# adityamwagh/SuperSLAM

Measured on AMD Instinct MI355X. Metric: stereo pairs/sec (SPx2+LG) at 1376x376, higher is better.
Workload: dtype f16; 1 GPU; configs[1]: SuperPoint x2 + select + gather + 1x LightGlue on 1376x376 stereo pairs; a step = 8 x 64 = 512 pairs per GPU resident in HBM (8 library calls of 64 pairs, different images per call), max_keypoints 600, seeded synthetic weights; pairs_per_call=64, max_keypoints=600, matches_last_call=1412, parallelism=replicated weights, pairs sharded over 1 rank(s), no data-path collective

## Files before the change

superslam_amd/csrc/api.hip:

```cpp
#include <algorithm>
#include <atomic>
#include <cmath>
#include <cstdarg>
#include <cstdlib>
#include <cstring>
#include <fstream>
#include <map>
#include <memory>
#include <mutex>
#include <string>
#include <vector>

#include "../../include/sship.h"
#include "../../include/superslam_hip/place_recognizer.hpp"
#include "kernels.h"

namespace sship {

static thread_local std::string g_err;
static void (*g_log_cb)(int, const char*) = nullptr;
static int g_profiling = 0;

void set_error(const std::string& msg) {
  g_err = msg;
// ... 508 lines not shown
  float* b1a = nullptr;
  _Float16* w1a_frag = nullptr;
  _Float16* w1a_fragb = nullptr;
  ConvW c1b, c2a, c2b, c3a, c3b, c4a, c4b, cPa, cPb, cDa, cDb;
  ConvW cDb32;
  sship_pool* pool = nullptr;
  int wsB = 0, wsH = 0, wsW = 0;
  DevBuf img, a1a, a1b, a2a, a2b, a3a, a3b, a4a, a4b, aPa, aDa, draw, logits, cand, cand_count;
  const void* cand_zero_ptr = nullptr; int cand_zero_n = 0;
  hipStream_t cand_zero_stream = nullptr;
  DevBuf kp, cell_h, cell_w, n_dev, desc_stage, gray_in;
  PinBuf h_kp, h_n, h_img;
  int cap = 0;
  float thr_f = 0.f;
  bool img_valid = false;
  struct Ring {
    int depth = 0, h = 0, w = 0, ch = 0;
    size_t img_bytes = 0;
    std::vector<void*> host, dev;
    std::vector<hipEvent_t> uploaded;
    hipStream_t copy_stream = nullptr;
    struct Pending { bool active = false; int slots[2] = {-1, -1}; int rc_pool = 0; hipEvent_t done = nullptr; void* h_kp = nullptr; void* h_n = nullptr; };
    std::vector<Pending> pending;
  } ring;
};

static void ring_free(sship_sp* sp);
static void sp_shapes(int H, int W, int& H2, int& W2, int& H4, int& W4, int& Hc, int& Wc) {
  H2 = H / 2; W2 = W / 2; H4 = H2 / 2; W4 = W2 / 2; Hc = H4 / 2; Wc = W4 / 2;
}

static int sp_ensure(sship_sp* sp, int B, int H, int W) {
  if (B <= sp->wsB && H == sp->wsH && W == sp->wsW) return SSHIP_OK;
  int H2, W2, H4, W4, Hc, Wc;
  sp_shapes(H, W, H2, W2, H4, W4, Hc, Wc);
  if (Hc < 1 || Wc < 1) return fail(SSHIP_ERR_INVALID, "image too small for SuperPoint (needs >= 8x8)");
  const size_t px1 = (size_t)B * H * W, px2 = (size_t)B * H2 * W2, px4 = (size_t)B * H4 * W4, pxc = (size_t)B * Hc * Wc;
  const int mk = sp->cfg.max_keypoints;
  SSHIP_HIP_CHECK(sp->img.ensure(px1));
  SSHIP_HIP_CHECK(sp->gray_in.ensure(px1 * 3));
  SSHIP_HIP_CHECK(sp->a1a.ensure(px1 * 64 * 2));
  SSHIP_HIP_CHECK(sp->a1b.ensure(px2 * 64 * 2));
  SSHIP_HIP_CHECK(sp->a2a.ensure(px2 * 64 * 2));
  SSHIP_HIP_CHECK(sp->a2b.ensure(px4 * 64 * 2));
  SSHIP_HIP_CHECK(sp->a3a.ensure(px4 * 128 * 2));
  SSHIP_HIP_CHECK(sp->a3b.ensure(pxc * 128 * 2));
  SSHIP_HIP_CHECK(sp->a4a.ensure(pxc * 128 * 2));
  SSHIP_HIP_CHECK(sp->a4b.ensure(pxc * 128 * 2));
  SSHIP_HIP_CHECK(sp->aPa.ensure(pxc * 256 * 2));
  SSHIP_HIP_CHECK(sp->aDa.ensure(pxc * 256 * 2));
  SSHIP_HIP_CHECK(sp->draw.ensure(pxc * 256 * 2));
  SSHIP_HIP_CHECK(sp->logits.ensure(pxc * kLogitStride * 4));
  sp->cap = Hc * 8 * Wc * 8;
  SSHIP_HIP_CHECK(sp->cand.ensure((size_t)B * sp->cap * 8));
  SSHIP_HIP_CHECK(sp->cand_count.ensure((size_t)B * 4));
  SSHIP_HIP_CHECK(sp->kp.ensure((size_t)B * mk * 3 * 4));
  SSHIP_HIP_CHECK(sp->cell_h.ensure((size_t)B * mk * 4));
  SSHIP_HIP_CHECK(sp->cell_w.ensure((size_t)B * mk * 4));
  SSHIP_HIP_CHECK(sp->n_dev.ensure((size_t)B * 4));
  SSHIP_HIP_CHECK(sp->h_kp.ensure((size_t)B * mk * 3 * 4));
  SSHIP_HIP_CHECK(sp->h_n.ensure((size_t)B * 4));
  SSHIP_HIP_CHECK(sp->h_img.ensure(px1 * 3));
  sp->wsB = B; sp->wsH = H; sp->wsW = W;
  return SSHIP_OK;
// ... 3 lines not shown
  static const int v = [] {
    const char* e = dev_env("SUPERSLAM_HIP_CONV");
    return (SSHIP_DEV_SWITCHES && e && std::string(e) == "strip") ? 2 : 1;
  }();
  return v;
}
static hipError_t conv3(const ConvW& w, const _Float16* in, _Float16* out, int B, int H, int W, bool pool, hipStream_t s) {
#if SSHIP_DEV_SWITCHES
  static const bool wino = [] { const char* e = dev_env("SUPERSLAM_HIP_CONV64"); return e && std::string(e) == "wino"; }();
  if (wino && w.w_wino && sp_conv3x3_wino_fits(H, W, w.cin, w.cout)) return sp_conv3x3_wino(w.w_wino, w.bias, in, out, B, H, W, pool, s);
  return conv_mode() == 1 ? sp_conv3x3_pp(w, in, out, B, H, W, pool, s) : sp_conv3x3_strip(w, in, out, B, H, W, pool, s);
#else
  return sp_conv3x3_pp(w, in, out, B, H, W, pool, s);
#endif
}
static bool conv2_fused(int B, int H2, int W2) {
#if SSHIP_DEV_SWITCHES
  static const std::string mode = [] { const char* e = dev_env("SUPERSLAM_HIP_CONV2"); return std::string(e ? e : ""); }();
  static const bool other = [] { const char* e = dev_env("SUPERSLAM_HIP_CONV64"); return e != nullptr; }();
  if (mode == "split" || other || conv_mode() != 1) return false;
#endif
  return sp_conv2ab_fused_fits(B, H2, W2, true);
}
static hipError_t conv3a_layer(const ConvW& w, const _Float16* in, _Float16* out, int B, int H, int W, hipStream_t s) {
#if SSHIP_DEV_SWITCHES
  static const bool roll = [] { const char* e = dev_env("SUPERSLAM_HIP_CONV3A"); return e && std::string(e) == "roll"; }();
  if (roll && conv_mode() == 1 && w.cin == 64 && w.cout == 128 && w.ct == 64 && sp_conv3a_roll_fits(B, H, W)) return sp_conv3a_roll(w, in, out, B, H, W, s);
#endif
  return conv3(w, in, out, B, H, W, false, s);
}
// ... 24 lines not shown
    g_timer.mark_fine("sp_gpu_infer:encoder/conv2a+conv2b+pool", s);
  } else {
    SSHIP_HIP_CHECK(conv3(sp->c2a, sp->a1b.as<_Float16>(), sp->a2a.as<_Float16>(), B, H2, W2, false, s));
    g_timer.mark_fine("sp_gpu_infer:encoder/conv2a", s);
    SSHIP_HIP_CHECK(conv3(sp->c2b, sp->a2a.as<_Float16>(), sp->a2b.as<_Float16>(), B, H2, W2, true, s));
    g_timer.mark_fine("sp_gpu_infer:encoder/conv2b+pool", s);
  }
  SSHIP_HIP_CHECK(conv3a_layer(sp->c3a, sp->a2b.as<_Float16>(), sp->a3a.as<_Float16>(), B, H4, W4, s));
  g_timer.mark_fine("sp_gpu_infer:encoder/conv3a", s);
  SSHIP_HIP_CHECK(conv3(sp->c3b, sp->a3a.as<_Float16>(), sp->a3b.as<_Float16>(), B, H4, W4, true, s));
  g_timer.mark_fine("sp_gpu_infer:encoder/conv3b+pool", s);
  SSHIP_HIP_CHECK(conv3(sp->c4a, sp->a3b.as<_Float16>(), sp->a4a.as<_Float16>(), B, Hc, Wc, false, s));
  g_timer.mark_fine("sp_gpu_infer:encoder/conv4a", s);
  SSHIP_HIP_CHECK(conv3(sp->c4b, sp->a4a.as<_Float16>(), sp->a4b.as<_Float16>(), B, Hc, Wc, false, s));
  g_timer.mark(g_profiling >= 2 ? "sp_gpu_infer:encoder/conv4b" : "sp_gpu_infer:encoder", s);
  SSHIP_HIP_CHECK(conv3(sp->cPa, sp->a4b.as<_Float16>(), sp->aPa.as<_Float16>(), B, Hc, Wc, false, s));
  g_timer.mark_fine("sp_gpu_infer:heads/convPa", s);
  SSHIP_HIP_CHECK(sp_conv1x1_f32(sp->cPb, sp->aPa.as<_Float16>(), sp->logits.as<float>(), kLogitStride, B, Hc, Wc, s));
  if (dense_desc || desc_dense_mode()) SSHIP_HIP_CHECK(conv3(sp->cDa, sp->a4b.as<_Float16>(), sp->aDa.as<_Float16>(), B, Hc, Wc, false, s));
  if (dense_desc) SSHIP_HIP_CHECK(sp_conv1x1_f16(sp->cDb, sp->aDa.as<_Float16>(), sp->draw.as<_Float16>(), B, Hc, Wc, s));
  g_timer.mark(g_profiling >= 2 ? "sp_gpu_infer:heads/convPb" : "sp_gpu_infer:heads", s);
  return SSHIP_OK;
}

static int sp_select(sship_sp* sp, int B, int H, int W, float* scores_out, float* kp_out, int* n_out, hipStream_t s) {
  int H2, W2, H4, W4, Hc, Wc;
  sp_shapes(H, W, H2, W2, H4, W4, Hc, Wc);
  if (sp->cand_zero_ptr != sp->cand_count.p || sp->cand_zero_n < B || sp->cand_zero_stream != s)
    SSHIP_HIP_CHECK(hipMemsetAsync(sp->cand_count.p, 0, (size_t)B * 4, s));
  sp->cand_zero_ptr = sp->cand_count.p; sp->cand_zero_n = 0; sp->cand_zero_stream = s;
  NmsArgs a{};
  a.logits = sp->logits.as<float>(); a.ls = kLogitStride; a.B = B; a.H = Hc * 8; a.W = Wc * 8;
  a.radius = sp->cfg.nms_radius; a.thr_f = sp->thr_f; a.border = sp->cfg.remove_borders;
  a.cand = sp->cand.as<unsigned long long>(); a.cand_count = sp->cand_count.as<int>(); a.cap = sp->cap;
  a.scores_out = scores_out;
  launch_nms_tile(0, a, s);
// ... 178 lines not shown
  SSHIP_HIP_CHECK(mfma_probe(random_operands != 0, tflops));
  return SSHIP_OK;
}

extern "C" int sship_sp_bench_layer(sship_sp* sp, int layer, int batch, int h, int w, int iters, float* avg_ms,
                                    double* macs) {
  bind_thread();
  if (!sp || !avg_ms || iters <= 0 || layer < 0 || layer > 15) return fail(SSHIP_ERR_INVALID, "sp_bench_layer: bad arguments");
  if (batch > sp->wsB || h != sp->wsH || w != sp->wsW) return fail(SSHIP_ERR_INVALID, "sp_bench_layer: run the network at this shape first");
  if (layer <= 1 && !sp->img_valid)
    return fail(SSHIP_ERR_INVALID, "sp_bench_layer: the handle holds no copy of the last input - make one call with sship_set_profiling(1) first "
                                   "(a launch on stale / zero pixels runs at a higher clock than the real one)");
  int H2, W2, H4, W4, Hc, Wc;
  sp_shapes(h, w, H2, W2, H4, W4, Hc, Wc);
  hipStream_t s = sp->stream;
  _Float16 *a1a = sp->a1a.as<_Float16>(), *a1b = sp->a1b.as<_Float16>(), *a2a = sp->a2a.as<_Float16>(),
           *a2b = sp->a2b.as<_Float16>(), *a3a = sp->a3a.as<_Float16>(), *a3b = sp->a3b.as<_Float16>(),
           *a4a = sp->a4a.as<_Float16>(), *a4b = sp->a4b.as<_Float16>(), *aPa = sp->aPa.as<_Float16>(),
           *aDa = sp->aDa.as<_Float16>();
  auto run = [&]() -> hipError_t {
    switch (layer) {
      case 0: launch_conv1a(sp->img.as<uint8_t>(), sp->w1a, sp->b1a, a1a, batch, h, w, s); return hipGetLastError();
      case 1: return conv1ab(sp, sp->img.as<uint8_t>(), a1b, batch, h, w, s);
      case 15:
        if (!sp_conv2ab_fused_fits(batch, H2, W2, true)) return hipErrorInvalidValue;
        return sp_conv2ab_fused(sp->c2a, sp->c2b, a1b, a2b, batch, H2, W2, s);
      case 2: return conv3(sp->c2a, a1b, a2a, batch, H2, W2, false, s);
      case 3: return conv3(sp->c2b, a2a, a2b, batch, H2, W2, true, s);
      case 4: return conv3a_layer(sp->c3a, a2b, a3a, batch, H4, W4, s);
      case 5: return conv3(sp->c3b, a3a, a3b, batch, H4, W4, true, s);
      case 6: return conv3(sp->c4a, a3b, a4a, batch, Hc, Wc, false, s);
      case 7: return conv3(sp->c4b, a4a, a4b, batch, Hc, Wc, false, s);
      case 8: return conv3(sp->cPa, a4b, aPa, batch, Hc, Wc, false, s);
      case 9: return sp_conv1x1_f32(sp->cPb, aPa, sp->logits.as<float>(), kLogitStride, batch, Hc, Wc, s);
      case 10: return conv3(sp->cDa, a4b, aDa, batch, Hc, Wc, false, s);
      case 11: return sp_conv1x1_f16(sp->cDb, aDa, sp->draw.as<_Float16>(), batch, Hc, Wc, s);
      case 12: {
        if (hipError_t e = hipMemsetAsync(sp->cand_count.p, 0, (size_t)batch * 4, s)) return e;
        sp->cand_zero_n = 0;
        NmsArgs a{};
        a.logits = sp->logits.as<float>(); a.ls = kLogitStride; a.B = batch; a.H = Hc * 8; a.W = Wc * 8;
        a.radius = sp->cfg.nms_radius; a.thr_f = sp->thr_f; a.border = sp->cfg.remove_borders;
        a.cand = sp->cand.as<unsigned long long>(); a.cand_count = sp->cand_count.as<int>(); a.cap = sp->cap;
        launch_nms_tile(0, a, s);
        return hipGetLastError();
      }
      case 13: {
        TopkArgs t{};
// ... 1010 lines not shown
```

superslam_amd/csrc/conv_pp128.hip:

```cpp
#include "igemm.h"
#include "kernels.h"

#include <cstdio>
#include <cstdlib>
#include <string>
#include <type_traits>
#include <vector>

#ifndef SSHIP_PP_PRIO
#define SSHIP_PP_PRIO 2
#endif
#ifndef SSHIP_PP_TRACE_BUILD
#define SSHIP_PP_TRACE_BUILD 0
#endif

#ifndef SSHIP_PP128_ABL
#define SSHIP_PP128_ABL 0
#endif
#ifndef SSHIP_PP128_COLMAJOR
#define SSHIP_PP128_COLMAJOR 0
#endif

namespace sship {

struct Pp128Args {
  const _Float16* in;
  const _Float16* wpack;
  const float* bias;
  _Float16* out;
  int B, H, W, cout;
  unsigned long long* trace;
  int pairs_on;
};

constexpr int Q_TH = 8, Q_TW = 32, Q_THH = 10, Q_TWH = 34;
constexpr int Q_IN_HALFS = Q_THH * Q_TWH * 32;
constexpr int Q_W_SLOT = 9 * 2 * 2 * 512;
constexpr int Q_ROW_UNITS = Q_TWH * 4;
constexpr int Q_NCHUNK = 4;
constexpr unsigned Q_OOB = 0xfffffff0u;

__device__ __forceinline__ int pp128_lds(int row, int col, int unit) {
  return (row * Q_TWH + col) * 32 + ((unit ^ ((col >> 2) & 3)) << 3);
}

struct TileWalk { int tx, ty, b; };

// ... 292 lines not shown
    std::vector<unsigned long long> h(4096 * 2 * 6);
    (void)hipStreamSynchronize(s);
    (void)hipMemcpy(h.data(), tbuf, h.size() * 8, hipMemcpyDeviceToHost);
    double sum[6] = {0}; long cnt = 0;
    for (int i = 0; i < gx * ncb * 2; ++i) {
      if (!h[i * 6 + 3]) continue;
      for (int k = 0; k < 6; ++k) sum[k] += (double)h[i * 6 + k];
      ++cnt;
    }
    if (cnt) fprintf(stderr, "[pp128 trace cout=%d pool=%d] weight dma issue=%.0f stage+dma wait=%.0f prefetch issue=%.0f | mfma=%.0f | barrier wait after data=%.0f after mfma=%.0f (clk, %ld groups)\n",
                     a.cout, (int)POOL, sum[0] / cnt, sum[1] / cnt, sum[2] / cnt, sum[3] / cnt, sum[4] / cnt, sum[5] / cnt, cnt);
  }
  return hipGetLastError();
}

constexpr int R_TH = 16, R_THH = 18;
constexpr int R_IN_UNITS = R_THH * Q_TWH * 4;
constexpr int R_IN_DMA = (R_IN_UNITS + 63) / 64;
constexpr int R_IN_HALFS = R_IN_DMA * 64 * 8;
constexpr int R_DMA_PER_WAVE = 10;
constexpr unsigned R_OOB = 0x80000000u;

typedef int rsrc4_t __attribute__((ext_vector_type(4)));

__host__ __device__ inline bool pp128w_pairs_shape(bool pool, int B, int W) {
  const int we = W - ((W + Q_TW - 1) / Q_TW - 1) * Q_TW;
  return !pool && (B & 1) == 0 && W > Q_TW && we >= 1 && we <= 15;
}
#define pp128w_pairs(pool, B, W) (p.pairs_on && pp128w_pairs_shape(pool, B, W))
template <bool POOL, int NCH>
__global__ __launch_bounds__(512, 2) void conv3x3_pp128w(Pp128Args p) {
  constexpr int MT = 2, NT = 4;
  constexpr int PB = NCH * 64;
  extern __shared__ __attribute__((aligned(16))) char smem128w[];
  _Float16* s_w = reinterpret_cast<_Float16*>(smem128w);
  const int tid = threadIdx.x, wave = tid >> 6, lane = tid & 63, j = lane & 31, hh = lane >> 5;
  const int grp = __builtin_amdgcn_readfirstlane(wave >> 2);
  const int gw = wave & 3;
  const int gw_u = __builtin_amdgcn_readfirstlane(gw);
  _Float16* my_in = s_w + 2 * Q_W_SLOT + grp * R_IN_HALFS;
  float* s_bias = reinterpret_cast<float*>(s_w + 2 * Q_W_SLOT + 2 * R_IN_HALFS);

  const int tiles_x = (p.W + Q_TW - 1) / Q_TW, tiles_y = (p.H + R_TH - 1) / R_TH;
  const bool pairs = pp128w_pairs(POOL, p.B, p.W);
  const int txn = tiles_x - 1, we = p.W - txn * Q_TW;
  const int tiles_xv = pairs ? 2 * txn + 1 : tiles_x, nb_walk = pairs ? p.B / 2 : p.B;
  const int ntiles = nb_walk * tiles_xv * tiles_y;
  const int cb = blockIdx.y;
  const int t_begin = (int)((long long)blockIdx.x * ntiles / gridDim.x);
  const int t_end = (int)((long long)(blockIdx.x + 1) * ntiles / gridDim.x);
  const int n_wg = t_end - t_begin;
  if (n_wg <= 0) return;
  const _Float16* wsrc = p.wpack + (size_t)cb * (NCH * Q_W_SLOT);

  for (int u = tid; u < (NCH == 2 ? 2 : 1) * Q_W_SLOT / 8; u += 512) *reinterpret_cast<uint4*>(s_w + u * 8) = *reinterpret_cast<const uint4*>(wsrc + u * 8);
  if (tid < 256) s_bias[tid] = p.bias[cb * 64 + (tid & 63)];
  const unsigned lane16 = lane * 16;
  const int dma_f0 = gw_u < 2 ? gw_u * 5 : 10 + (gw_u - 2) * 4;
  auto fill_weights = [&](int cn, int half) __attribute__((always_inline)) {
    const unsigned long long ga = (unsigned long long)(uintptr_t)(wsrc + (size_t)cn * Q_W_SLOT + (half * 18 + dma_f0) * 512);
    const unsigned long long g = (unsigned long long)(unsigned)__builtin_amdgcn_readfirstlane((unsigned)ga) |
                                 ((unsigned long long)(unsigned)__builtin_amdgcn_readfirstlane((unsigned)(ga >> 32)) << 32);
    const unsigned dst = __builtin_amdgcn_readfirstlane((unsigned)(uintptr_t)(s_w + (cn & 1) * Q_W_SLOT + (half * 18 + dma_f0) * 512));
    unsigned keep;
    asm volatile("s_mov_b32 %0, m0\n\ts_mov_b32 m0, %2\n\ts_nop 0\n\t"
                 "global_load_lds_dwordx4 %1, %3\n\t"
                 "global_load_lds_dwordx4 %1, %3 offset:1024\n\t"
                 "global_load_lds_dwordx4 %1, %3 offset:2048\n\t"
                 "global_load_lds_dwordx4 %1, %3 offset:3072\n\t"
                 "s_mov_b32 m0, %0"
                 : "=&s"(keep) : "v"(lane16), "s"(dst), "s"(g) : "memory");
// ... 75 lines not shown
    rs[3] = 0x00020000;
  }
  const unsigned lds_in0 = __builtin_amdgcn_readfirstlane((unsigned)(uintptr_t)(my_in + (gw_u * R_DMA_PER_WAVE) * 512));
  auto dma_tile = [&](const TileWalk& w, int chunk, unsigned m0a, unsigned m0b, unsigned m0c) __attribute__((always_inline)) {
    int img, txr;
    bool shared;
    decode(w, img, txr, shared);
    const int y0 = w.ty * R_TH, x0 = txr * Q_TW;
    const unsigned soff = __builtin_amdgcn_readfirstlane((unsigned)((img * p.H + y0) * p.W + x0) * (unsigned)PB + (unsigned)chunk * 64u);
    const bool interior = !shared && y0 >= 1 && y0 + R_TH + 1 <= p.H && x0 >= 1 && x0 + Q_TW + 1 <= p.W;
    unsigned v[R_DMA_PER_WAVE];
    if (interior) {
#pragma unroll
      for (int i = 0; i < R_DMA_PER_WAVE; ++i) v[i] = voff[i];
    } else if (shared) {
      unsigned ok = 0x3ffu & ~m_dead;
      if (w.ty == 0) ok &= m_top;
      if (w.ty == tiles_y - 1) ok &= m_bot;
      const unsigned delta = (unsigned)(p.H * p.W - (we + 2)) * (unsigned)PB;
#pragma unroll
      for (int i = 0; i < R_DMA_PER_WAVE; ++i) v[i] = (ok >> i) & 1u ? voff[i] + ((m_second >> i) & 1u ? delta : 0u) : R_OOB;
    } else {
      unsigned ok = 0x3ffu;
      if (w.ty == 0) ok &= m_top;
      if (w.ty == tiles_y - 1) ok &= m_bot;
      if (txr == 0) ok &= m_left;
      if (txr == tiles_x - 1) ok &= m_right;
#pragma unroll
      for (int i = 0; i < R_DMA_PER_WAVE; ++i) v[i] = (ok >> i) & 1u ? voff[i] : R_OOB;
    }
    unsigned keep;
    asm volatile("s_mov_b32 %0, m0\n\ts_mov_b32 m0, %5\n\ts_nop 0\n\t"
                 "buffer_load_dwordx4 %1, %6, %7 offen lds\n\t"
                 "buffer_load_dwordx4 %2, %6, %7 offen offset:1024 lds\n\t"
                 "buffer_load_dwordx4 %3, %6, %7 offen offset:2048 lds\n\t"
                 "buffer_load_dwordx4 %4, %6, %7 offen offset:3072 lds\n\t"
                 "s_mov_b32 m0, %0"
                 : "=&s"(keep) : "v"(v[0]), "v"(v[1]), "v"(v[2]), "v"(v[3]), "s"(m0a), "s"(rs), "s"(soff) : "memory");
    asm volatile("s_mov_b32 %0, m0\n\ts_mov_b32 m0, %5\n\ts_nop 0\n\t"
                 "buffer_load_dwordx4 %1, %6, %7 offen lds\n\t"
                 "buffer_load_dwordx4 %2, %6, %7 offen offset:1024 lds\n\t"
                 "buffer_load_dwordx4 %3, %6, %7 offen offset:2048 lds\n\t"
                 "buffer_load_dwordx4 %4, %6, %7 offen offset:3072 lds\n\t"
                 "s_mov_b32 m0, %0"
                 : "=&s"(keep) : "v"(v[4]), "v"(v[5]), "v"(v[6]), "v"(v[7]), "s"(m0b), "s"(rs), "s"(soff) : "memory");
    if (gw_u < 3)
      asm volatile("s_mov_b32 %0, m0\n\ts_mov_b32 m0, %3\n\ts_nop 0\n\t"
                   "buffer_load_dwordx4 %1, %4, %5 offen lds\n\t"
                   "buffer_load_dwordx4 %2, %4, %5 offen offset:1024 lds\n\t"
                   "s_mov_b32 m0, %0"
                   : "=&s"(keep) : "v"(v[8]), "v"(v[9]), "s"(m0c), "s"(rs), "s"(soff) : "memory");
    else
      asm volatile("s_mov_b32 %0, m0\n\ts_mov_b32 m0, %2\n\ts_nop 0\n\t"
                   "buffer_load_dwordx4 %1, %3, %4 offen lds\n\t"
                   "s_mov_b32 m0, %0"
                   : "=&s"(keep) : "v"(v[8]), "s"(m0c), "s"(rs), "s"(soff) : "memory");
  };
  auto dma_in = [&](int chunk) __attribute__((always_inline)) {
    dma_tile(pw, chunk, lds_in0, lds_in0 + 4096u, lds_in0 + 8192u);
    if (chunk == NCH - 1) walk_next(pw);
  };

  f16x_t acc[MT][NT];
  auto mfma_item = [&](auto chunk_c) __attribute__((always_inline)) {
    constexpr int chunk = decltype(chunk_c)::value;
    const _Float16* wc = s_w + (chunk & 1) * Q_W_SLOT + lane * 8;
    const _Float16* ib = my_in + (gw * 4) * Q_TWH * 32;
    h8_t af[3][MT], rows[8];
    auto load_a = [&](int s_, int buf) __attribute__((always_inline)) {
      const int t = s_ / 3, ky = s_ - 3 * t, kx = t >> 1, ksl = t & 1, idx = (ky * 3 + kx) * 2 + ksl;
#pragma unroll
      for (int m = 0; m < MT; ++m) af[buf][m] = *reinterpret_cast<const h8_t*>(wc + (idx * MT + m) * 512);
    };
    auto load_row = [&](int t, int row) __attribute__((always_inline)) {
      rows[(6 * t + row) & 7] = *reinterpret_cast<const h8_t*>(ib + row * Q_TWH * 32 + boff[t >> 1][t & 1]);
    };
#pragma unroll
    for (int row = 0; row < 4; ++row) load_row(0, row);
    load_a(0, 0);
    load_a(1, 1);
    if constexpr (chunk == 0) {
#pragma unroll
      for (int m = 0; m < MT; ++m)
#pragma unroll
        for (int n = 0; n < NT; ++n)
#pragma unroll
          for (int g = 0; g < 4; ++g) {
            const float4 b4 = *reinterpret_cast<const float4*>(s_bias + n * 64 + m * 32 + hh * 4 + g * 8);
            acc[m][n][4 * g + 0] = b4.x; acc[m][n][4 * g + 1] = b4.y; acc[m][n][4 * g + 2] = b4.z; acc[m][n][4 * g + 3] = b4.w;
          }
    }
    if constexpr ((SSHIP_PP128_ABL & 8) != 0) {
      load_a(2, 2);
#pragma unroll
      for (int row = 4; row < 8; ++row) rows[row] = rows[row - 4];
    }
#pragma unroll
    for (int s_ = 0; s_ < 18; ++s_) {
      const int t = s_ / 3, ky = s_ - 3 * t;
      if constexpr ((SSHIP_PP128_ABL & 8) == 0) {
      if (s_ + 2 < 18) load_a(s_ + 2, (s_ + 2) % 3);
      if (ky == 0) {
        load_row(t, 4); load_row(t, 5);
        if (t + 1 < 6) { load_row(t + 1, 0); load_row(t + 1, 1); }
      } else if (t + 1 < 6) load_row(t + 1, ky + 1);
      }
      __builtin_amdgcn_sched_barrier(0);
#pragma unroll
      for (int n = 0; n < NT; ++n)
#pragma unroll
        for (int m = 0; m < MT; ++m) {
          if constexpr ((SSHIP_PP128_ABL & 1) != 0) asm volatile("" :: "v"(af[s_ % 3][m]), "v"(rows[(6 * t + n + ky) & 7]));
          else acc[m][n] = mfma32(af[s_ % 3][m], rows[(6 * t + n + ky) & 7], acc[m][n]);
        }
      __builtin_amdgcn_sched_barrier(0);
    }
  };
  auto epilogue = [&]() __attribute__((always_inline)) {
    int b, txr;
    bool shared;
    decode(ew, b, txr, shared);
    const int y0 = ew.ty * R_TH, x0 = txr * Q_TW;
    walk_next(ew);
    const int yb = y0 + gw * 4;
    int x = x0 + j;
    if (shared) {
      const bool second = j >= we + 2;
      b += second;
// ... 41 lines not shown
        auto pool1 = [&](int m, int r) __attribute__((always_inline)) -> float {
          const float tt = fmaxf(fmaxf(acc[m][2 * q][r], acc[m][2 * q + 1][r]), 0.f);
          const float nb = __int_as_float(__builtin_amdgcn_update_dpp(0, __float_as_int(tt), 0xB1, 0xF, 0xF, false));
          return fmaxf(tt, nb);
        };
#pragma unroll
        for (int m = 0; m < MT; ++m)
#pragma unroll
          for (int g = 0; g < 4; g += 2)
            store_pair(pix, m, g, pack2(pool1(m, 4 * g + 0), pool1(m, 4 * g + 1)), pack2(pool1(m, 4 * g + 2), pool1(m, 4 * g + 3)),
                       pack2(pool1(m, 4 * g + 4), pool1(m, 4 * g + 5)), pack2(pool1(m, 4 * g + 6), pool1(m, 4 * g + 7)), ok);
      }
    }
  };

  const int T0 = (n_wg + 1) >> 1, T1 = n_wg >> 1;
  unsigned long long* trow = p.trace + ((size_t)(blockIdx.y * gridDim.x + blockIdx.x) * 2 + grp) * 6;
  const bool tr_lane = SSHIP_PP_TRACE_BUILD && p.trace && gw == 0 && lane == 0;
  unsigned long long t0 = 0, t1 = 0;
  auto data_role = [&](int dma_chunk, int dma_half, int in_chunk, bool tr) __attribute__((always_inline)) {
    if (SSHIP_PP_PRIO) __builtin_amdgcn_s_setprio(SSHIP_PP_PRIO);
    if (tr) t0 = __builtin_readcyclecounter();
    if constexpr ((SSHIP_PP128_ABL & 2) != 0) {
      if (in_chunk >= 0 && in_chunk == NCH - 1) walk_next(pw);
    } else {
    if (in_chunk >= 0) dma_in(in_chunk);
    if (NCH == 4 && dma_chunk >= 0) fill_weights(dma_chunk, dma_half);
    }
    if (SSHIP_PP_PRIO) __builtin_amdgcn_s_setprio(0);
    if (tr) { t1 = __builtin_readcyclecounter(); trow[0] = t1 - t0; t0 = t1; }
    asm volatile("s_waitcnt vmcnt(0)" ::: "memory");
    if (tr) { t1 = __builtin_readcyclecounter(); trow[1] = t1 - t0; trow[2] = 0; t0 = t1; }
    __syncthreads();
    if (tr) trow[4] = __builtin_readcyclecounter() - t0;
  };
  auto mfma_role = [&](auto chunk_c, bool tr) __attribute__((always_inline)) {
    constexpr int chunk = decltype(chunk_c)::value;
    if (tr) t0 = __builtin_readcyclecounter();
    mfma_item(chunk_c);
    if constexpr (chunk == NCH - 1) {
      if constexpr ((SSHIP_PP128_ABL & 4) != 0) {
        walk_next(ew);
#pragma unroll
        for (int m = 0; m < MT; ++m)
#pragma unroll
          for (int n = 0; n < NT; ++n) asm volatile("" :: "v"(acc[m][n]));
      } else epilogue();
    }
    if (tr) { t1 = __builtin_readcyclecounter(); trow[3] = t1 - t0; t0 = t1; }
    __syncthreads();
    if (tr) trow[5] = __builtin_readcyclecounter() - t0;
  };
  const std::integral_constant<int, 0> c0{};
  const std::integral_constant<int, 1> c1{};
  const std::integral_constant<int, 2> c2{};
  const std::integral_constant<int, 3> c3{};
  __syncthreads();
  if constexpr (NCH == 4) {
    if (grp == 0) {
      data_role(-1, 0, T0 > 0 ? 0 : -1, false);
#pragma unroll 1
      for (int it = 0; it < T0; ++it) {
        const bool more = it + 1 < T0, tr = tr_lane && it == 1;
        mfma_role(c0, tr);
        data_role(1, 1, 1, tr);
        mfma_role(c1, false);
        data_role(2, 1, 2, false);
        mfma_role(c2, false);
        data_role(3, 1, 3, false);
        mfma_role(c3, false);
        data_role(0, 1, more ? 0 : -1, false);
      }
    } else {
// ... 76 lines not shown
    std::vector<unsigned long long> h(4096 * 2 * 6);
    (void)hipStreamSynchronize(s);
    (void)hipMemcpy(h.data(), tbuf, h.size() * 8, hipMemcpyDeviceToHost);
    double sum[6] = {0}; long cnt = 0;
    for (int i = 0; i < gx * ncb * 2; ++i) {
      if (!h[i * 6 + 3]) continue;
      for (int k = 0; k < 6; ++k) sum[k] += (double)h[i * 6 + k];
      ++cnt;
    }
    if (cnt) fprintf(stderr, "[pp128w trace cin=%d cout=%d pool=%d] dma issue=%.0f dma wait=%.0f | mfma=%.0f | barrier wait after data=%.0f after mfma=%.0f (clk, %ld groups)\n",
                     NCH * 32, a.cout, (int)POOL, sum[0] / cnt, sum[1] / cnt, sum[3] / cnt, sum[4] / cnt, sum[5] / cnt, cnt);
  }
  return hipGetLastError();
}

bool sp_conv3x3_pp128_fits(int B, int H, int W, int cin) { return (size_t)B * H * W * cin * 2 + (size_t)(W + 1) * cin * 4 + 8192 < 0x7f000000ull; }

hipError_t sp_conv3x3_pp128(const ConvW& w, const _Float16* in, _Float16* out, int B, int H, int W, bool pool, hipStream_t s) {
  if ((w.cin != 128 && w.cin != 64) || !w.w_q || w.cout % 64 || !sp_conv3x3_pp128_fits(B, H, W, w.cin)) return hipErrorInvalidValue;
  Pp128Args a{};
  a.in = in; a.wpack = w.w_q; a.bias = w.bias; a.out = out; a.B = B; a.H = H; a.W = W; a.cout = w.cout;
  if (w.cin == 64) return pool ? launch_pp128w<true, 2>(a, s) : launch_pp128w<false, 2>(a, s);
  static const bool th8 = [] { const char* e = dev_env("SUPERSLAM_HIP_CONV128"); return e && std::string(e) == "th8"; }();
  if (th8) return pool ? launch_pp128<true>(a, s) : launch_pp128<false>(a, s);
  return pool ? launch_pp128w<true, 4>(a, s) : launch_pp128w<false, 4>(a, s);
}

}
```

superslam_amd/csrc/kernels.h:

```cpp
#pragma once
#include "common.h"

namespace sship {

constexpr int kMaxKp = 4096;
constexpr int kLogitStride = 68;

void launch_conv1a(const uint8_t* img, const float* w, const float* bias, _Float16* out, int B, int H, int W,
                   hipStream_t s);
struct NmsArgs {
  const float* logits;
  int ls;
  const float* scores_in;
  int B, H, W;
  int radius;
  float thr_f;
  int border;
  unsigned long long* cand;
  int* cand_count;
  int cap;
  float* scores_out;
  float* scores_raw_out;
};
float threshold_as_float(double thr);
// ... 27 lines not shown

struct ConvW {
  _Float16* w = nullptr;
  _Float16* w_wino = nullptr;
  _Float16* w_q = nullptr;
  float* bias = nullptr;
  int cin = 0, cout = 0, cout_pad = 0, ks = 1, ct = 64;
};
hipError_t sp_conv3x3_strip(const ConvW& w, const _Float16* in, _Float16* out, int B, int H, int W, bool pool,
                            hipStream_t s);
hipError_t sp_conv1ab_fused(const ConvW& w1b, const _Float16* w1a_frag, const float* b1a, const uint8_t* img,
                            _Float16* out, int B, int H, int W, hipStream_t s);
hipError_t sp_conv3x3_pp(const ConvW& w, const _Float16* in, _Float16* out, int B, int H, int W, bool pool, hipStream_t s);
bool sp_conv3x3_pp128_fits(int B, int H, int W, int cin);
hipError_t sp_conv3x3_pp128(const ConvW& w, const _Float16* in, _Float16* out, int B, int H, int W, bool pool, hipStream_t s);
bool sp_conv2ab_fused_fits(int B, int H, int W, bool any_batch);
hipError_t sp_conv2ab_fused(const ConvW& wa, const ConvW& wb, const _Float16* in, _Float16* out, int B, int H, int W, hipStream_t s);
bool sp_conv3a_roll_fits(int B, int H, int W);
hipError_t sp_conv3a_roll(const ConvW& w, const _Float16* in, _Float16* out, int B, int H, int W, hipStream_t s);
hipError_t sp_conv1ab_pp(const ConvW& w1b, const _Float16* w1a_frag, const float* b1a, const uint8_t* img, _Float16* out,
                         int B, int H, int W, hipStream_t s);
bool sp_conv3x3_wino_fits(int H, int W, int cin, int cout);
hipError_t sp_conv3x3_wino(const _Float16* upack, const float* bias, const _Float16* in, _Float16* out, int B, int H, int W, bool pool, hipStream_t s);
hipError_t sp_conv1x1_f16(const ConvW& w, const _Float16* in, _Float16* out, int B, int H, int W, hipStream_t s);
int cu_count();

hipError_t mfma_probe(bool random_operands, float* tflops);

hipError_t launch_desc_head_sparse(const ConvW& da32, const ConvW& db32, const _Float16* a4b, int Hc, int Wc, const int* cell_h,
                                   const int* cell_w, const int* n_dev, int max_kp, int B, _Float16* out, size_t out_img_stride,
// ... 44 lines not shown
```

Before: 5765 pairs/s.

## Fuse SuperPoint detector head convPa and 1x1 convPb into one kernel

Adds a HEAD variant of the pp128w 3x3 conv kernel that computes convPa (128->256) and applies ReLU and the 65-channel 1x1 convPb in its epilogue using MFMA on register-held tiles, writing logits directly. The 256-channel intermediate activation never goes to HBM, and one launch is removed. To fit the extra LDS and accumulators, the tile height is halved (8 rows) and the kernel loops over four output-channel blocks per tile, re-streaming the input each pass. This may reduce parallelism and add redundant input traffic.

New measurement: 5825 pairs/s, median of 6. 1.0% higher.

```diff
diff --git a/superslam_amd/csrc/api.hip b/superslam_amd/csrc/api.hip
--- a/superslam_amd/csrc/api.hip
+++ b/superslam_amd/csrc/api.hip
@@ -546,6 +546,7 @@
   int cap = 0;
   float thr_f = 0.f;
   bool img_valid = false;
+  bool pa_valid = false;
   struct Ring {
     int depth = 0, h = 0, w = 0, ch = 0;
     size_t img_bytes = 0;
@@ -562,6 +563,7 @@
   H2 = H / 2; W2 = W / 2; H4 = H2 / 2; W4 = W2 / 2; Hc = H4 / 2; Wc = W4 / 2;
 }
 
+static bool head_fused(int B, int Hc, int Wc);
 static int sp_ensure(sship_sp* sp, int B, int H, int W) {
   if (B <= sp->wsB && H == sp->wsH && W == sp->wsW) return SSHIP_OK;
   int H2, W2, H4, W4, Hc, Wc;
@@ -579,7 +581,7 @@
   SSHIP_HIP_CHECK(sp->a3b.ensure(pxc * 128 * 2));
   SSHIP_HIP_CHECK(sp->a4a.ensure(pxc * 128 * 2));
   SSHIP_HIP_CHECK(sp->a4b.ensure(pxc * 128 * 2));
-  SSHIP_HIP_CHECK(sp->aPa.ensure(pxc * 256 * 2));
+  if (!head_fused(B, Hc, Wc)) SSHIP_HIP_CHECK(sp->aPa.ensure(pxc * 256 * 2));
   SSHIP_HIP_CHECK(sp->aDa.ensure(pxc * 256 * 2));
   SSHIP_HIP_CHECK(sp->draw.ensure(pxc * 256 * 2));
   SSHIP_HIP_CHECK(sp->logits.ensure(pxc * kLogitStride * 4));
@@ -613,6 +615,18 @@
   return sp_conv3x3_pp(w, in, out, B, H, W, pool, s);
 #endif
 }
+static bool head_fused(int B, int Hc, int Wc) {
+#if SSHIP_DEV_SWITCHES
+  static const bool split = [] {
+    const char* h = dev_env("SUPERSLAM_HIP_HEAD");
+    const char* c = dev_env("SUPERSLAM_HIP_CONV128");
+    const char* p = dev_env("SUPERSLAM_HIP_CONVPB");
+    return (h && std::string(h) == "split") || c || p;
+  }();
+  if (split || conv_mode() != 1) return false;
+#endif
+  return sp_conv_head_pb_fits(B, Hc, Wc);
+}
 static bool conv2_fused(int B, int H2, int W2) {
 #if SSHIP_DEV_SWITCHES
   static const std::string mode = [] { const char* e = dev_env("SUPERSLAM_HIP_CONV2"); return std::string(e ? e : ""); }();
@@ -667,12 +681,20 @@
   g_timer.mark_fine("sp_gpu_infer:encoder/conv4a", s);
   SSHIP_HIP_CHECK(conv3(sp->c4b, sp->a4a.as<_Float16>(), sp->a4b.as<_Float16>(), B, Hc, Wc, false, s));
   g_timer.mark(g_profiling >= 2 ? "sp_gpu_infer:encoder/conv4b" : "sp_gpu_infer:encoder", s);
-  SSHIP_HIP_CHECK(conv3(sp->cPa, sp->a4b.as<_Float16>(), sp->aPa.as<_Float16>(), B, Hc, Wc, false, s));
-  g_timer.mark_fine("sp_gpu_infer:heads/convPa", s);
-  SSHIP_HIP_CHECK(sp_conv1x1_f32(sp->cPb, sp->aPa.as<_Float16>(), sp->logits.as<float>(), kLogitStride, B, Hc, Wc, s));
+  const bool fused_head = head_fused(B, Hc, Wc);
+  if (fused_head) {
+    SSHIP_HIP_CHECK(sp_conv_head_pb(sp->cPa, sp->cPb, sp->a4b.as<_Float16>(), sp->logits.as<float>(), B, Hc, Wc, s));
+    sp->pa_valid = false;
+  } else {
+    SSHIP_HIP_CHECK(sp->aPa.ensure((size_t)B * Hc * Wc * 256 * 2));
+    SSHIP_HIP_CHECK(conv3(sp->cPa, sp->a4b.as<_Float16>(), sp->aPa.as<_Float16>(), B, Hc, Wc, false, s));
+    g_timer.mark_fine("sp_gpu_infer:heads/convPa", s);
+    SSHIP_HIP_CHECK(sp_conv1x1_f32(sp->cPb, sp->aPa.as<_Float16>(), sp->logits.as<float>(), kLogitStride, B, Hc, Wc, s));
+    sp->pa_valid = true;
+  }
   if (dense_desc || desc_dense_mode()) SSHIP_HIP_CHECK(conv3(sp->cDa, sp->a4b.as<_Float16>(), sp->aDa.as<_Float16>(), B, Hc, Wc, false, s));
   if (dense_desc) SSHIP_HIP_CHECK(sp_conv1x1_f16(sp->cDb, sp->aDa.as<_Float16>(), sp->draw.as<_Float16>(), B, Hc, Wc, s));
-  g_timer.mark(g_profiling >= 2 ? "sp_gpu_infer:heads/convPb" : "sp_gpu_infer:heads", s);
+  g_timer.mark(g_profiling < 2 ? "sp_gpu_infer:heads" : fused_head ? "sp_gpu_infer:heads/convPa+convPb" : "sp_gpu_infer:heads/convPb", s);
   return SSHIP_OK;
 }
 
@@ -881,6 +903,11 @@
   int H2, W2, H4, W4, Hc, Wc;
   sp_shapes(h, w, H2, W2, H4, W4, Hc, Wc);
   hipStream_t s = sp->stream;
+  if (layer == 8 || layer == 9) {
+    if (layer == 9 && !sp->pa_valid)
+      return fail(SSHIP_ERR_INVALID, "sp_bench_layer: no convPa map on this handle (the detector head ran fused) - bench layer 8 first");
+    SSHIP_HIP_CHECK(sp->aPa.ensure((size_t)sp->wsB * Hc * Wc * 256 * 2));
+  }
   _Float16 *a1a = sp->a1a.as<_Float16>(), *a1b = sp->a1b.as<_Float16>(), *a2a = sp->a2a.as<_Float16>(),
            *a2b = sp->a2b.as<_Float16>(), *a3a = sp->a3a.as<_Float16>(), *a3b = sp->a3b.as<_Float16>(),
            *a4a = sp->a4a.as<_Float16>(), *a4b = sp->a4b.as<_Float16>(), *aPa = sp->aPa.as<_Float16>(),
@@ -898,7 +925,7 @@
       case 5: return conv3(sp->c3b, a3a, a3b, batch, H4, W4, true, s);
       case 6: return conv3(sp->c4a, a3b, a4a, batch, Hc, Wc, false, s);
       case 7: return conv3(sp->c4b, a4a, a4b, batch, Hc, Wc, false, s);
-      case 8: return conv3(sp->cPa, a4b, aPa, batch, Hc, Wc, false, s);
+      case 8: sp->pa_valid = true; return conv3(sp->cPa, a4b, aPa, batch, Hc, Wc, false, s);
       case 9: return sp_conv1x1_f32(sp->cPb, aPa, sp->logits.as<float>(), kLogitStride, batch, Hc, Wc, s);
       case 10: return conv3(sp->cDa, a4b, aDa, batch, Hc, Wc, false, s);
       case 11: return sp_conv1x1_f16(sp->cDb, aDa, sp->draw.as<_Float16>(), batch, Hc, Wc, s);
diff --git a/superslam_amd/csrc/conv_pp128.hip b/superslam_amd/csrc/conv_pp128.hip
--- a/superslam_amd/csrc/conv_pp128.hip
+++ b/superslam_amd/csrc/conv_pp128.hip
@@ -31,6 +31,9 @@
   int B, H, W, cout;
   unsigned long long* trace;
   int pairs_on;
+  const _Float16* pbw;
+  const float* pbb;
+  float* logits;
 };
 
 constexpr int Q_TH = 8, Q_TW = 32, Q_THH = 10, Q_TWH = 34;
@@ -353,11 +356,16 @@
   return hipGetLastError();
 }
 
-constexpr int R_TH = 16, R_THH = 18;
-constexpr int R_IN_UNITS = R_THH * Q_TWH * 4;
-constexpr int R_IN_DMA = (R_IN_UNITS + 63) / 64;
-constexpr int R_IN_HALFS = R_IN_DMA * 64 * 8;
-constexpr int R_DMA_PER_WAVE = 10;
+template <bool PB>
+struct PpGeo {
+  static constexpr int TH = PB ? 8 : 16, THH = TH + 2;
+  static constexpr int IN_UNITS = THH * Q_TWH * 4;
+  static constexpr int IN_DMA = (IN_UNITS + 63) / 64;
+  static constexpr int IN_HALFS = IN_DMA * 64 * 8;
+  static constexpr int DMA_PER_WAVE = PB ? 6 : 10;
+};
+constexpr int R_TH = PpGeo<false>::TH, R_THH = PpGeo<false>::THH;
+constexpr int R_IN_HALFS = PpGeo<false>::IN_HALFS;
 constexpr unsigned R_OOB = 0x80000000u;
 
 typedef int rsrc4_t __attribute__((ext_vector_type(4)));
@@ -367,9 +375,11 @@
   return !pool && (B & 1) == 0 && W > Q_TW && we >= 1 && we <= 15;
 }
 #define pp128w_pairs(pool, B, W) (p.pairs_on && pp128w_pairs_shape(pool, B, W))
-template <bool POOL, int NCH>
+template <bool POOL, int NCH, bool HEAD = false>
 __global__ __launch_bounds__(512, 2) void conv3x3_pp128w(Pp128Args p) {
-  constexpr int MT = 2, NT = 4;
+  using G = PpGeo<HEAD>;
+  constexpr int R_TH = G::TH, R_THH = G::THH, R_IN_HALFS = G::IN_HALFS, R_DMA_PER_WAVE = G::DMA_PER_WAVE;
+  constexpr int MT = 2, NT = R_TH / 4;
   constexpr int PB = NCH * 64;
   extern __shared__ __attribute__((aligned(16))) char smem128w[];
   _Float16* s_w = reinterpret_cast<_Float16*>(smem128w);
@@ -379,6 +389,8 @@
   const int gw_u = __builtin_amdgcn_readfirstlane(gw);
   _Float16* my_in = s_w + 2 * Q_W_SLOT + grp * R_IN_HALFS;
   float* s_bias = reinterpret_cast<float*>(s_w + 2 * Q_W_SLOT + 2 * R_IN_HALFS);
+  _Float16* s_pbw = reinterpret_cast<_Float16*>(s_bias + 512);
+  float* s_pbb = reinterpret_cast<float*>(s_pbw + 8 * 5 * 512);
 
   const int tiles_x = (p.W + Q_TW - 1) / Q_TW, tiles_y = (p.H + R_TH - 1) / R_TH;
   const bool pairs = pp128w_pairs(POOL, p.B, p.W);
@@ -393,7 +405,16 @@
   const _Float16* wsrc = p.wpack + (size_t)cb * (NCH * Q_W_SLOT);
 
   for (int u = tid; u < (NCH == 2 ? 2 : 1) * Q_W_SLOT / 8; u += 512) *reinterpret_cast<uint4*>(s_w + u * 8) = *reinterpret_cast<const uint4*>(wsrc + u * 8);
-  if (tid < 256) s_bias[tid] = p.bias[cb * 64 + (tid & 63)];
+  if constexpr (HEAD) {
+    s_bias[tid] = p.bias[(tid >> 7) * 64 + (tid & 63)];
+    for (int u = tid; u < 8 * 5 * 64; u += 512) {
+      const int ks = u / 320, r = u - ks * 320, mb = r >> 6, l = r & 63;
+      *reinterpret_cast<uint4*>(s_pbw + u * 8) = *reinterpret_cast<const uint4*>(p.pbw + (size_t)(16 * mb + (l & 15)) * 256 + ks * 32 + (l >> 4) * 8);
+    }
+    if (tid < 80) s_pbb[tid] = tid < 65 ? p.pbb[tid] : 0.f;
+  } else {
+    if (tid < 256) s_bias[tid] = p.bias[cb * 64 + (tid & 63)];
+  }
   const unsigned lane16 = lane * 16;
   const int dma_f0 = gw_u < 2 ? gw_u * 5 : 10 + (gw_u - 2) * 4;
   auto fill_weights = [&](int cn, int half) __attribute__((always_inline)) {
@@ -499,14 +520,14 @@
 #pragma unroll
       for (int i = 0; i < R_DMA_PER_WAVE; ++i) v[i] = voff[i];
     } else if (shared) {
-      unsigned ok = 0x3ffu & ~m_dead;
+      unsigned ok = ((1u << R_DMA_PER_WAVE) - 1u) & ~m_dead;
       if (w.ty == 0) ok &= m_top;
       if (w.ty == tiles_y - 1) ok &= m_bot;
       const unsigned delta = (unsigned)(p.H * p.W - (we + 2)) * (unsigned)PB;
 #pragma unroll
       for (int i = 0; i < R_DMA_PER_WAVE; ++i) v[i] = (ok >> i) & 1u ? voff[i] + ((m_second >> i) & 1u ? delta : 0u) : R_OOB;
     } else {
-      unsigned ok = 0x3ffu;
+      unsigned ok = (1u << R_DMA_PER_WAVE) - 1u;
       if (w.ty == 0) ok &= m_top;
       if (w.ty == tiles_y - 1) ok &= m_bot;
       if (txr == 0) ok &= m_left;
@@ -522,6 +543,15 @@
                  "buffer_load_dwordx4 %4, %6, %7 offen offset:3072 lds\n\t"
                  "s_mov_b32 m0, %0"
                  : "=&s"(keep) : "v"(v[0]), "v"(v[1]), "v"(v[2]), "v"(v[3]), "s"(m0a), "s"(rs), "s"(soff) : "memory");
+    if constexpr (HEAD) {
+      if (gw_u < 3)
+        asm volatile("s_mov_b32 %0, m0\n\ts_mov_b32 m0, %3\n\ts_nop 0\n\t"
+                     "buffer_load_dwordx4 %1, %4, %5 offen lds\n\t"
+                     "buffer_load_dwordx4 %2, %4, %5 offen offset:1024 lds\n\t"
+                     "s_mov_b32 m0, %0"
+                     : "=&s"(keep) : "v"(v[4]), "v"(v[5]), "s"(m0b), "s"(rs), "s"(soff) : "memory");
+      return;
+    } else {
     asm volatile("s_mov_b32 %0, m0\n\ts_mov_b32 m0, %5\n\ts_nop 0\n\t"
                  "buffer_load_dwordx4 %1, %6, %7 offen lds\n\t"
                  "buffer_load_dwordx4 %2, %6, %7 offen offset:1024 lds\n\t"
@@ -540,17 +570,19 @@
                    "buffer_load_dwordx4 %1, %3, %4 offen lds\n\t"
                    "s_mov_b32 m0, %0"
                    : "=&s"(keep) : "v"(v[8]), "s"(m0c), "s"(rs), "s"(soff) : "memory");
-  };
-  auto dma_in = [&](int chunk) __attribute__((always_inline)) {
+    }
+  };
+  auto dma_in = [&](int chunk, bool last_pass) __attribute__((always_inline)) {
     dma_tile(pw, chunk, lds_in0, lds_in0 + 4096u, lds_in0 + 8192u);
-    if (chunk == NCH - 1) walk_next(pw);
+    if (chunk == NCH - 1 && last_pass) walk_next(pw);
   };
 
   f16x_t acc[MT][NT];
-  auto mfma_item = [&](auto chunk_c) __attribute__((always_inline)) {
+  auto slot = [](int t, int row) { return NT == 4 ? (6 * t + row) & 7 : (4 * t + row) & 7; };
+  auto mfma_item = [&](auto chunk_c, const float* bias) __attribute__((always_inline)) {
     constexpr int chunk = decltype(chunk_c)::value;
     const _Float16* wc = s_w + (chunk & 1) * Q_W_SLOT + lane * 8;
-    const _Float16* ib = my_in + (gw * 4) * Q_TWH * 32;
+    const _Float16* ib = my_in + (gw * NT) * Q_TWH * 32;
     h8_t af[3][MT], rows[8];
     auto load_a = [&](int s_, int buf) __attribute__((always_inline)) {
       const int t = s_ / 3, ky = s_ - 3 * t, kx = t >> 1, ksl = t & 1, idx = (ky * 3 + kx) * 2 + ksl;
@@ -558,7 +590,7 @@
       for (int m = 0; m < MT; ++m) af[buf][m] = *reinterpret_cast<const h8_t*>(wc + (idx * MT + m) * 512);
     };
     auto load_row = [&](int t, int row) __attribute__((always_inline)) {
-      rows[(6 * t + row) & 7] = *reinterpret_cast<const h8_t*>(ib + row * Q_TWH * 32 + boff[t >> 1][t & 1]);
+      rows[slot(t, row)] = *reinterpret_cast<const h8_t*>(ib + row * Q_TWH * 32 + boff[t >> 1][t & 1]);
     };
 #pragma unroll
     for (int row = 0; row < 4; ++row) load_row(0, row);
@@ -571,7 +603,7 @@
         for (int n = 0; n < NT; ++n)
 #pragma unroll
           for (int g = 0; g < 4; ++g) {
-            const float4 b4 = *reinterpret_cast<const float4*>(s_bias + n * 64 + m * 32 + hh * 4 + g * 8);
+            const float4 b4 = *reinterpret_cast<const float4*>(bias + n * 64 + m * 32 + hh * 4 + g * 8);
             acc[m][n][4 * g + 0] = b4.x; acc[m][n][4 * g + 1] = b4.y; acc[m][n][4 * g + 2] = b4.z; acc[m][n][4 * g + 3] = b4.w;
           }
     }
@@ -585,18 +617,24 @@
       const int t = s_ / 3, ky = s_ - 3 * t;
       if constexpr ((SSHIP_PP128_ABL & 8) == 0) {
       if (s_ + 2 < 18) load_a(s_ + 2, (s_ + 2) % 3);
+      if constexpr (NT == 4) {
       if (ky == 0) {
         load_row(t, 4); load_row(t, 5);
         if (t + 1 < 6) { load_row(t + 1, 0); load_row(t + 1, 1); }
       } else if (t + 1 < 6) load_row(t + 1, ky + 1);
+      } else {
+        if (ky == 0 && t + 1 < 6)
+#pragma unroll
+          for (int row = 0; row < 4; ++row) load_row(t + 1, row);
+      }
       }
       __builtin_amdgcn_sched_barrier(0);
 #pragma unroll
       for (int n = 0; n < NT; ++n)
 #pragma unroll
         for (int m = 0; m < MT; ++m) {
-          if constexpr ((SSHIP_PP128_ABL & 1) != 0) asm volatile("" :: "v"(af[s_ % 3][m]), "v"(rows[(6 * t + n + ky) & 7]));
-          else acc[m][n] = mfma32(af[s_ % 3][m], rows[(6 * t + n + ky) & 7], acc[m][n]);
+          if constexpr ((SSHIP_PP128_ABL & 1) != 0) asm volatile("" :: "v"(af[s_ % 3][m]), "v"(rows[slot(t, n + ky)]));
+          else acc[m][n] = mfma32(af[s_ % 3][m], rows[slot(t, n + ky)], acc[m][n]);
         }
       __builtin_amdgcn_sched_barrier(0);
     }
@@ -668,17 +706,91 @@
     }
   };
 
+  typedef float f4x_t __attribute__((ext_vector_type(4)));
+  f4x_t pacc[HEAD ? NT : 1][2][5];
+  auto epilogue_pb = [&](int cbp) __attribute__((always_inline)) {
+    const int kb = lane >> 4;
+    if (cbp == 0) {
+#pragma unroll
+      for (int n = 0; n < NT; ++n)
+#pragma unroll
+        for (int q = 0; q < 2; ++q)
+#pragma unroll
+          for (int mb = 0; mb < 5; ++mb) pacc[n][q][mb] = *reinterpret_cast<const f4x_t*>(s_pbb + 16 * mb + 4 * kb);
+    }
+    const h2_t z2 = {(_Float16)0.f, (_Float16)0.f};
+    auto relu2 = [&](float lo, float hi) __attribute__((always_inline)) -> unsigned {
+      h2_t v = {(_Float16)lo, (_Float16)hi};
+      v = __builtin_elementwise_max(v, z2);
+      return *reinterpret_cast<const unsigned*>(&v);
+    };
+#pragma unroll
+    for (int n = 0; n < NT; ++n)
+#pragma unroll
+      for (int m = 0; m < MT; ++m) {
+        const f16x_t& a = acc[m][n];
+        unsigned d[4][2];
+#pragma unroll
+        for (int g = 0; g < 4; ++g) { d[g][0] = relu2(a[4 * g + 0], a[4 * g + 1]); d[g][1] = relu2(a[4 * g + 2], a[4 * g + 3]); }
+        const auto x0 = __builtin_amdgcn_permlane32_swap(d[0][0], d[2][0], false, false);
+        const auto x1 = __builtin_amdgcn_permlane32_swap(d[0][1], d[2][1], false, false);
+        const auto y0 = __builtin_amdgcn_permlane32_swap(d[1][0], d[3][0], false, false);
+        const auto y1 = __builtin_amdgcn_permlane32_swap(d[1][1], d[3][1], false, false);
+        const unsigned X[4] = {x0[0], x1[0], x0[1], x1[1]}, Y[4] = {y0[0], y1[0], y0[1], y1[1]};
+        unsigned T[2][4];
+#pragma unroll
+        for (int k = 0; k < 4; ++k) {
+          const auto r = __builtin_amdgcn_permlane16_swap(X[k], Y[k], false, false);
+          T[0][k] = r[0]; T[1][k] = r[1];
+        }
+        const _Float16* wa = s_pbw + (cbp * 2 + m) * (5 * 512) + lane * 8;
+#pragma unroll
+        for (int q = 0; q < 2; ++q) {
+          const h8_t bq = *reinterpret_cast<const h8_t*>(T[q]);
+#pragma unroll
+          for (int mb = 0; mb < 5; ++mb)
+            pacc[n][q][mb] = __builtin_amdgcn_mfma_f32_16x16x32_f16(*reinterpret_cast<const h8_t*>(wa + mb * 512), bq, pacc[n][q][mb], 0, 0, 0);
+        }
+      }
+    if (cbp != Q_NCHUNK - 1) return;
+    int b, txr;
+    bool shared;
+    decode(ew, b, txr, shared);
+    const int y0 = ew.ty * R_TH, x0 = txr * Q_TW;
+    walk_next(ew);
+#pragma unroll
+    for (int q = 0; q < 2; ++q) {
+      const int jj = 16 * q + (lane & 15);
+      int bq = b, x = x0 + jj;
+      if (shared) {
+        const bool second = jj >= we + 2;
+        bq += second;
+        x = second ? x0 + jj - (we + 2) : (jj < we ? x : p.W);
+      }
+#pragma unroll
+      for (int n = 0; n < NT; ++n) {
+        const int y = y0 + gw * NT + n;
+        if (y < p.H && x < p.W) {
+          float* o = p.logits + ((size_t)(bq * p.H + y) * p.W + x) * kLogitStride + 4 * kb;
+#pragma unroll
+          for (int mb = 0; mb < 4; ++mb) *reinterpret_cast<f4x_t*>(o + 16 * mb) = pacc[n][q][mb];
+          if (kb == 0) o[64] = pacc[n][q][4][0];
+        }
+      }
+    }
+  };
+
   const int T0 = (n_wg + 1) >> 1, T1 = n_wg >> 1;
   unsigned long long* trow = p.trace + ((size_t)(blockIdx.y * gridDim.x + blockIdx.x) * 2 + grp) * 6;
   const bool tr_lane = SSHIP_PP_TRACE_BUILD && p.trace && gw == 0 && lane == 0;
   unsigned long long t0 = 0, t1 = 0;
-  auto data_role = [&](int dma_chunk, int dma_half, int in_chunk, bool tr) __attribute__((always_inline)) {
+  auto data_role = [&](int dma_chunk, int dma_half, int in_chunk, bool tr, bool last_pass = true) __attribute__((always_inline)) {
     if (SSHIP_PP_PRIO) __builtin_amdgcn_s_setprio(SSHIP_PP_PRIO);
     if (tr) t0 = __builtin_readcyclecounter();
     if constexpr ((SSHIP_PP128_ABL & 2) != 0) {
       if (in_chunk >= 0 && in_chunk == NCH - 1) walk_next(pw);
     } else {
-    if (in_chunk >= 0) dma_in(in_chunk);
+    if (in_chunk >= 0) dma_in(in_chunk, last_pass);
     if (NCH == 4 && dma_chunk >= 0) fill_weights(dma_chunk, dma_half);
     }
     if (SSHIP_PP_PRIO) __builtin_amdgcn_s_setprio(0);
@@ -688,12 +800,13 @@
     __syncthreads();
     if (tr) trow[4] = __builtin_readcyclecounter() - t0;
   };
-  auto mfma_role = [&](auto chunk_c, bool tr) __attribute__((always_inline)) {
+  auto mfma_role = [&](auto chunk_c, bool tr, int cbp = 0) __attribute__((always_inline)) {
     constexpr int chunk = decltype(chunk_c)::value;
     if (tr) t0 = __builtin_readcyclecounter();
-    mfma_item(chunk_c);
+    mfma_item(chunk_c, HEAD ? s_bias + cbp * 128 : s_bias);
     if constexpr (chunk == NCH - 1) {
-      if constexpr ((SSHIP_PP128_ABL & 4) != 0) {
+      if constexpr (HEAD) epilogue_pb(cbp);
+      else if constexpr ((SSHIP_PP128_ABL & 4) != 0) {
         walk_next(ew);
 #pragma unroll
         for (int m = 0; m < MT; ++m)
@@ -710,7 +823,51 @@
   const std::integral_constant<int, 2> c2{};
   const std::integral_constant<int, 3> c3{};
   __syncthreads();
-  if constexpr (NCH == 4) {
+  if constexpr (HEAD) {
+    if (grp == 0) {
+      data_role(-1, 0, T0 > 0 ? 0 : -1, false);
+#pragma unroll 1
+      for (int it = 0; it < T0; ++it) {
+        const bool more = it + 1 < T0;
+#pragma unroll 1
+        for (int cbp = 0; cbp < 4; ++cbp) {
+          const int cn = 4 * cbp;
+          mfma_role(c0, false, cbp);
+          data_role(cn + 1, 1, 1, false);
+          mfma_role(c1, false, cbp);
+          data_role(cn + 2, 1, 2, false);
+          mfma_role(c2, false, cbp);
+          data_role(cn + 3, 1, 3, false, cbp == 3);
+          mfma_role(c3, false, cbp);
+          data_role((cn + 4) & 15, 1, cbp < 3 || more ? 0 : -1, false);
+        }
+      }
+    } else {
+      __syncthreads();
+#pragma unroll 1
+      for (int it = 0; it < T1; ++it) {
+#pragma unroll 1
+        for (int cbp = 0; cbp < 4; ++cbp) {
+          const int cn = 4 * cbp;
+          data_role(cn + 1, 0, 0, false);
+          mfma_role(c0, false, cbp);
+          data_role(cn + 2, 0, 1, false);
+          mfma_role(c1, false, cbp);
+          data_role(cn + 3, 0, 2, false);
+          mfma_role(c2, false, cbp);
+          data_role((cn + 4) & 15, 0, 3, false, cbp == 3);
+          mfma_role(c3, false, cbp);
+        }
+      }
+      if (T0 > T1) {
+#pragma unroll 1
+        for (int c = 0; c < 16; ++c) {
+          data_role((c + 1) & 15, 0, -1, false);
+          __syncthreads();
+        }
+      }
+    }
+  } else if constexpr (NCH == 4) {
     if (grp == 0) {
       data_role(-1, 0, T0 > 0 ? 0 : -1, false);
 #pragma unroll 1
@@ -817,7 +974,30 @@
   return hipGetLastError();
 }
 
+hipError_t sp_conv_head_pb(const ConvW& pa, const ConvW& pb, const _Float16* in, float* logits, int B, int H, int W, hipStream_t s) {
+  if (pa.cin != 128 || pa.cout != 256 || !pa.w_q || pb.cin != 256 || pb.cout != 65 || !pb.w_q || !sp_conv_head_pb_fits(B, H, W))
+    return hipErrorInvalidValue;
+  using G = PpGeo<true>;
+  constexpr size_t smem = (size_t)(2 * Q_W_SLOT + 2 * G::IN_HALFS) * 2 + 512 * 4 + 8 * 5 * 512 * 2 + 80 * 4;
+  static_assert(smem <= 163840, "LDS budget");
+  auto kern = conv3x3_pp128w<false, 4, true>;
+  static const hipError_t attr_rc = hipFuncSetAttribute(reinterpret_cast<const void*>(kern), hipFuncAttributeMaxDynamicSharedMemorySize, (int)smem);
+  if (attr_rc != hipSuccess) return attr_rc;
+  static const bool pairs_env = !(dev_env("SUPERSLAM_HIP_CONV128_PAIRS") && atoi(dev_env("SUPERSLAM_HIP_CONV128_PAIRS")) == 0);
+  const bool pairs = pairs_env && pp128w_pairs_shape(false, B, W);
+  const int tiles_x = (W + Q_TW - 1) / Q_TW;
+  const int ntiles = (pairs ? B / 2 * (2 * (tiles_x - 1) + 1) : B * tiles_x) * ((H + G::TH - 1) / G::TH);
+  int gx = cu_count();
+  if (gx * 2 > ntiles) gx = (ntiles + 1) / 2;
+  if (gx < 1) gx = 1;
+  Pp128Args a{};
+  a.in = in; a.wpack = pa.w_q; a.bias = pa.bias; a.out = nullptr; a.B = B; a.H = H; a.W = W; a.cout = pa.cout;
+  a.pbw = pb.w_q; a.pbb = pb.bias; a.logits = logits; a.pairs_on = pairs_env ? 1 : 0;
+  hipLaunchKernelGGL(kern, dim3(gx, 1), dim3(512), smem, s, a);
+  return hipGetLastError();
+}
 bool sp_conv3x3_pp128_fits(int B, int H, int W, int cin) { return (size_t)B * H * W * cin * 2 + (size_t)(W + 1) * cin * 4 + 8192 < 0x7f000000ull; }
+bool sp_conv_head_pb_fits(int B, int H, int W) { return sp_conv3x3_pp128_fits(B, H, W, 128); }
 
 hipError_t sp_conv3x3_pp128(const ConvW& w, const _Float16* in, _Float16* out, int B, int H, int W, bool pool, hipStream_t s) {
   if ((w.cin != 128 && w.cin != 64) || !w.w_q || w.cout % 64 || !sp_conv3x3_pp128_fits(B, H, W, w.cin)) return hipErrorInvalidValue;
diff --git a/superslam_amd/csrc/kernels.h b/superslam_amd/csrc/kernels.h
--- a/superslam_amd/csrc/kernels.h
+++ b/superslam_amd/csrc/kernels.h
@@ -65,6 +65,8 @@
 hipError_t sp_conv3x3_pp(const ConvW& w, const _Float16* in, _Float16* out, int B, int H, int W, bool pool, hipStream_t s);
 bool sp_conv3x3_pp128_fits(int B, int H, int W, int cin);
 hipError_t sp_conv3x3_pp128(const ConvW& w, const _Float16* in, _Float16* out, int B, int H, int W, bool pool, hipStream_t s);
+bool sp_conv_head_pb_fits(int B, int H, int W);
+hipError_t sp_conv_head_pb(const ConvW& pa, const ConvW& pb, const _Float16* in, float* logits, int B, int H, int W, hipStream_t s);
 bool sp_conv2ab_fused_fits(int B, int H, int W, bool any_batch);
 hipError_t sp_conv2ab_fused(const ConvW& wa, const ConvW& wb, const _Float16* in, _Float16* out, int B, int H, int W, hipStream_t s);
 bool sp_conv3a_roll_fits(int B, int H, int W);
```
